# JohannesBuchner/massivedatans

Hardware: AMD Instinct MI355X
Metric: likelihood evals/sec across N datasets per constrained draw (higher is better)
Workload: dtype f64

## Files before the change

massivedatans_amd/csrc/mdns_chunk.hip:

```cpp
#include "mdns_quad.h"
#include <cstdlib>

namespace mdns {

typedef JointMailbox ChunkMailbox;

template <int NST>
__global__ __launch_bounds__(256) void k_chunk_accept(
    const double *__restrict__ Y, int ld, int nx, int nxp, const double *__restrict__ xgrid,
    const double *__restrict__ params, int B, double scale,
    const int *__restrict__ rows, int *__restrict__ rows_dev, int M, int ntiles,
    const double *__restrict__ higher, int *__restrict__ flags, int stamp, JointTrail trail, JointHeader *__restrict__ header)
{
	extern __shared__ __attribute__((aligned(16))) double lds[];
	if (blockIdx.x == 0 && threadIdx.x == 0) header->status = 0;
	double2 *tpl = reinterpret_cast<double2 *>(lds);
	double *par = lds + (size_t) nxp * 4;
	unsigned long long *votes = reinterpret_cast<unsigned long long *>(par + 12);
	const int lane = threadIdx.x & 63, wave = threadIdx.x >> 6;
	const int q = lane & 3;
	const int bt = blockIdx.x / ntiles, tile = blockIdx.x - bt * ntiles;
	double pv = 0.0;
	if (threadIdx.x < 12) {
		const int b = bt * 4 + threadIdx.x / 3;
// ... 240 lines not shown
		const int kk = live ? k : M - 1;
		const int d = thr_rows ? thr_rows[kk] : kk;
		thr[v] = live ? higher[d] : __builtin_nan("");
		yy[v] = ysq[d];
	}
	int best = 0x7fffffff;
#pragma unroll
	for (int c = 0; c < NC; c++) {
		const int cand = (ct0 + c) * 16 + i;
		const bool valid = ct0 + c < nbt && cand < B;
		const double mm = msq[valid ? cand : 0];
		bool hit = false, maybe = false;
#pragma unroll
		for (int v = 0; v < 4; v++) {
			const double S = acc[c][v];
			const double Lf = scale * ((mm - 2.0 * S) + yy[v]);
			const double E4 = 4.0 * unit * ((mm + 2.0 * fabs(S)) + yy[v]);
			const bool h = valid && Lf > thr[v] + E4;
			hit = hit || h;
			maybe = maybe || (valid && !h && Lf >= thr[v] - E4);
		}
		const unsigned long long hm = __ballot(hit), mb = __ballot(maybe);
		if (lane < 16) {
			const unsigned long long mine = 0x0001000100010001ull << lane;
			if (hm & mine) { flags[cand] = 1; best = cand < best ? cand : best; }
			else if (mb & mine) ambiguous[cand] = stamp;
		}
	}
#pragma unroll
	for (int off = 8; off > 0; off >>= 1) { const int o = __shfl_xor(best, off, 64); best = o < best ? o : best; }
	if (lane == 0 && best != 0x7fffffff) atomicMax(lowest, B - best);
}

template <int NC, bool KSPLIT>
__global__ __launch_bounds__(256) void k_gauss_gemm_filter(
    const double *__restrict__ YG, int nxg, int nx, const double *__restrict__ model_g, const double *__restrict__ msq, int B,
    double scale, const int *__restrict__ thr_rows, int M, int nbt,
    const double *__restrict__ higher, const double *__restrict__ ysq, int *__restrict__ flags, int *__restrict__ ambiguous,
    int stamp, int *__restrict__ lowest)
{
	__shared__ double red[KSPLIT ? 3 : 1][KSPLIT ? NC * 256 : 1];
	const int lane = threadIdx.x & 63, wave = __builtin_amdgcn_readfirstlane((int) (threadIdx.x >> 6));
	const int i = lane & 15, q = lane >> 4;
	const int rtile = KSPLIT ? blockIdx.x : blockIdx.x * 4 + wave;
	const int first = rtile * 16;
	if (first >= M) return;
	const int ct0 = blockIdx.y * NC;
	const int ncp = nxg >> 1, ng = nxg >> 4;
	const int g0 = KSPLIT ? (wave * ng) >> 2 : 0, g1 = KSPLIT ? ((wave + 1) * ng) >> 2 : ng;
	const double *pa = YG + (((size_t) rtile * ncp + 2 * q) << 5) + 2 * i;
	const double *pb[NC];
#pragma unroll
	for (int c = 0; c < NC; c++) pb[c] = model_g + (((size_t) (ct0 + c < nbt ? ct0 + c : nbt - 1) * ncp + 2 * q) << 5) + 2 * i;
	double4_t acc[NC];
#pragma unroll
	for (int c = 0; c < NC; c++) acc[c] = double4_t{0, 0, 0, 0};
	double4_t a[2], b[2][NC];
#define GG_LOAD4(P, G) gg_join(*reinterpret_cast<const double2_t *>((P) + ((size_t) (G) << 8)), *reinterpret_cast<const double2_t *>((P) + ((size_t) (G) << 8) + 32))
#define GG_FETCH(SET, G) { \
	const int g_ = (G) < g1 ? (G) : g1 - 1; \
	a[SET] = GG_LOAD4(pa, g_); \
	_Pragma("unroll") for (int c = 0; c < NC; c++) b[SET][c] = GG_LOAD4(pb[c], g_); }
#define GG_BODY(SET, G) { \
	__builtin_amdgcn_sched_barrier(0); \
	if ((G) < g1) { \
		_Pragma("unroll") for (int t = 0; t < 4; t++) \
			_Pragma("unroll") for (int c = 0; c < NC; c++) \
				acc[c] = __builtin_amdgcn_mfma_f64_16x16x4f64(a[SET][t], b[SET][c][t], acc[c], 0, 0, 0); \
	} \
	__builtin_amdgcn_sched_barrier(0); }
	if (g0 < g1) {
		GG_FETCH(0, g0)
// ... 24 lines not shown
				acc[c][v] = ((acc[c][v] + red[0][(c * 4 + v) * 64 + lane]) + red[1][(c * 4 + v) * 64 + lane]) + red[2][(c * 4 + v) * 64 + lane];
	}
	const double unit = fabs(scale) * (double) (nx + 8) * 0x1p-52;
	double thr[4], yy[4];
#pragma unroll
	for (int v = 0; v < 4; v++) {
		const int k = first + 4 * v + q;
		const bool live = k < M;
		const int kk = live ? k : M - 1;
		const int d = thr_rows ? thr_rows[kk] : kk;
		thr[v] = live ? higher[d] : __builtin_nan("");
		yy[v] = ysq[d];
	}
	int best = 0x7fffffff;
#pragma unroll
	for (int c = 0; c < NC; c++) {
		const int cand = (ct0 + c) * 16 + i;
		const bool valid = ct0 + c < nbt && cand < B;
		const double mm = msq[valid ? cand : 0];
		bool hit = false, maybe = false;
#pragma unroll
		for (int v = 0; v < 4; v++) {
			const double S = acc[c][v];
			const double Lf = scale * ((mm - 2.0 * S) + yy[v]);
			const double E4 = 4.0 * unit * ((mm + 2.0 * fabs(S)) + yy[v]);
			const bool h = valid && Lf > thr[v] + E4;
			hit = hit || h;
			maybe = maybe || (valid && !h && Lf >= thr[v] - E4);
		}
		const unsigned long long hm = __ballot(hit), mb = __ballot(maybe);
		if (lane < 16) {
			const unsigned long long mine = 0x0001000100010001ull << lane;
			if (hm & mine) { flags[cand] = 1; best = cand < best ? cand : best; }
			else if (mb & mine) ambiguous[cand] = stamp;
		}
	}
#pragma unroll
	for (int off = 8; off > 0; off >>= 1) { const int o = __shfl_xor(best, off, 64); best = o < best ? o : best; }
	if (lane == 0 && best != 0x7fffffff) atomicMax(lowest, B - best);
}

static constexpr int kExactMost = 64;
template <int NST>
__global__ __launch_bounds__(256) void k_exact_list(
    const double *__restrict__ Y, int ld, int nxp, const double *__restrict__ model_t, double scale,
    const int *__restrict__ rows, int M, int ntiles, const double *__restrict__ higher, int B,
    const int *__restrict__ ambiguous, int stamp, const int *__restrict__ lowest, int *__restrict__ flags, JointTrail trail,
    JointHeader *__restrict__ header)
{
	extern __shared__ __attribute__((aligned(16))) double lds[];
	double2 *tpl = reinterpret_cast<double2 *>(lds);
	unsigned long long *votes = reinterpret_cast<unsigned long long *>(lds + (size_t) nxp * 4);
	__shared__ int list[kExactMost];
	__shared__ int s_n;
	const int lane = threadIdx.x & 63, wave = threadIdx.x >> 6;
	if (wave == 0) {
		const int low = *lowest > 0 ? B - *lowest : B;
		int n = 0;
		for (int b0 = 0; b0 < B && b0 <= low; b0 += 64) {
			const int b = b0 + lane;
			const bool take = b < B && ((b < low && ambiguous[b] == stamp) || b == low);
			const unsigned long long m = __ballot(take);
			if (take) {
				const int at = n + __popcll(m & ((1ull << lane) - 1ull));
				if (at < kExactMost) list[at] = b;
			}
			n += __popcll(m);
		}
		if (lane == 0) {
			s_n = n < kExactMost ? n : kExactMost;
			if (n > kExactMost && blockIdx.x == 0) atomicOr(&header->status, 2);
		}
	}
	__syncthreads();
	const int n = s_n;
	if (n == 0) return;
	const int q = lane & 3;
	const int tile = blockIdx.x;
	const int r = wave * 16 + (lane >> 2);
	const int k = tile * 64 + r;
	const bool live = k < M;
	const int kk = live ? k : M - 1;
	const int row = rows ? rows[kk] : kk;
	double2 y[NST];
	const double thr = quad_load_row<NST>(Y, ld, row, live, q, higher, y);
	for (int g = 0; g < n; g += 4) {
		quad_templates_listed(lds, model_t, nxp, list, g, n);
		__syncthreads();
		const double L = quad_sum<NST>(tpl, nxp / kCH, q, y) * scale;
		const bool has_q = g + q < n, has_w = g + wave < n;
		quad_vote(L, thr, has_q, has_q ? list[g + q] : -1, has_w, has_w ? list[g + wave] : -1, ntiles, tile, r, votes, flags, 1, trail);
		__syncthreads();
	}
}

bool chunk_fits(const mdns_spectra *s, int M, int B)
{
	Context *c = ctx();
	const int ntiles = (M + 63) / 64;
	const long long groups = (long long) ntiles * ((B + 3) / 4);
	static const char *limit = getenv("MDNS_CHUNK_GROUPS");
	const long long most = limit && atoll(limit) > 0 ? atoll(limit) : 16LL * c->num_cus;
	if (M > 4096 && B > 8) return false;
	return groups <= most && cols_nx(s->nx) <= 8 * 32 && s->d_x != nullptr;
}

bool launch_chunk_accept(const mdns_spectra *s, const double *d_params_mapped, int B, double scale,
                         const int *d_rows_in, int *d_rows_dev, int M, const double *d_higher,
                         int *d_flags, int stamp, const JointTrail &trail, void *d_header)
{
	Context *c = ctx();
	const int ntiles = (M + 63) / 64;
	const int nbt = (B + 3) / 4;
	const int nxp = cols_nx(s->nx);
	const size_t lds = ((size_t) nxp * 4 + 12 + 4) * sizeof(double);
	const int nst = nxp / kCH;
	ProfileScope prof(0);
#define CHUNK_LAUNCH(NST) hipLaunchKernelGGL((k_chunk_accept<NST>), dim3(ntiles * nbt), dim3(256), lds, c->stream, \
	s->d_y, s->ld, s->nx, nxp, s->d_x, d_params_mapped, B, scale, d_rows_in, d_rows_dev, M, ntiles, d_higher, d_flags, stamp, trail, (JointHeader *) d_header)
	if (nst <= 8) { note_kernel(0, "k_chunk_accept<8>"); CHUNK_LAUNCH(8); }
	else if (nst <= 16) { note_kernel(0, "k_chunk_accept<16>"); CHUNK_LAUNCH(16); }
	else if (nst <= 26) { note_kernel(0, "k_chunk_accept<26>"); CHUNK_LAUNCH(26); }
	else { note_kernel(0, "k_chunk_accept<32>"); CHUNK_LAUNCH(32); }
#undef CHUNK_LAUNCH
	return launched("k_chunk_accept");
}

bool launch_chunk_commit(const int *d_thr_rows, int M, int B, const int *d_flags, int stamp, const JointTrail &trail,
                         const JointArrays &st, void *d_header, unsigned long long *d_fillbits, void *box_dev,
                         unsigned long long seq)
{
	Context *c = ctx();
	const int ntiles = (M + 63) / 64;
	hipLaunchKernelGGL(k_chunk_commit, dim3(1), dim3(1024), 0, c->stream, d_thr_rows, M, B, ntiles, d_flags, stamp, trail, st,
	                   (JointHeader *) d_header, d_fillbits, (ChunkMailbox *) box_dev, seq);
	return launched("k_chunk_commit");
}

int gauss_mfma_form()
{
	static int form = -1;
	if (form < 0) {
		const char *e = getenv("MDNS_K1_FILTER_FORM");
		form = e && e[0] == 'd' ? 1 : (e && e[0] == 'l' ? 0 : 2);
	}
	return form;
}

bool launch_gauss_mfma_filter(const mdns_spectra *s, const double *d_yT, const double *d_model_t, int B, double scale,
                              const int *d_thr_rows, int M, const double *d_higher, int *d_flags,
                              const double *d_msq, const JointTrail &trail, int *d_lowest, int *d_scratch, void *d_header,
                              const double *d_yG, const double *d_model_g)
{
	Context *c = ctx();
	const int ntiles = (M + 63) / 64, nbt = (B + 15) / 16;
	const int nxp = cols_nx(s->nx);
	int *d_amb = d_scratch;
	{
		static const char *probe = getenv("MDNS_FILTER_PROBE");
		const int pr = probe ? atoi(probe) : 0;
		if (pr == 0 && d_yG && d_model_g && gauss_mfma_form() == 2) {
			const int nxg = tiled16_nx(s->nx);
			static const char *ncf = getenv("MDNS_K1_GEMM_NC");
			int nc = nbt >= 2 ? 2 : 1;
			if (ncf && (atoi(ncf) == 1 || atoi(ncf) == 2 || atoi(ncf) == 4) && atoi(ncf) <= nbt) nc = atoi(ncf);
			ProfileScope prof(0);
			note_kernel(0, "k_gauss_gemm_filter<%d>", nc);
			static const char *ks = getenv("MDNS_K1_GEMM_KSPLIT");
			const bool ksplit = ks && ks[0] == '1';
			const int rt = (M + 15) / 16;
#define GG_LAUNCH(NC) do { if (ksplit) hipLaunchKernelGGL((k_gauss_gemm_filter<NC, true>), dim3(rt, (nbt + NC - 1) / NC), dim3(256), 0, c->stream, \
			d_yG, nxg, s->nx, d_model_g, d_msq, B, scale, d_thr_rows, M, nbt, d_higher, (const double *) s->d_ysq, d_flags, d_amb, trail.stamp, d_lowest); \
		else hipLaunchKernelGGL((k_gauss_gemm_filter<NC, false>), dim3((rt + 3) / 4, (nbt + NC - 1) / NC), dim3(256), 0, c->stream, \
			d_yG, nxg, s->nx, d_model_g, d_msq, B, scale, d_thr_rows, M, nbt, d_higher, (const double *) s->d_ysq, d_flags, d_amb, trail.stamp, d_lowest); } while (0)
			if (nc == 4) GG_LAUNCH(4); else if (nc == 2) GG_LAUNCH(2); else GG_LAUNCH(1);
#undef GG_LAUNCH
			if (!launched("k_gauss_gemm_filter")) return false;
		} else if (pr == 0 && gauss_mfma_form() == 1) {
			static double *d_zeros = nullptr;
			if (!d_zeros && (!MDNS_HIP(hipMalloc((void **) &d_zeros, 16 * sizeof(double))) ||
			                 !MDNS_HIP(hipMemsetAsync(d_zeros, 0, 16 * sizeof(double), c->stream)))) return false;
			const int nc = nbt >= 16 ? 4 : (nbt >= 8 ? 2 : 1);
			const int gy = (nbt + 4 * nc - 1) / (4 * nc);
			ProfileScope prof(0);
			note_kernel(0, "k_gauss_mfma_direct<%d>", nc);
#define GD_LAUNCH(NC) hipLaunchKernelGGL((k_gauss_mfma_direct<NC>), dim3((M + 15) / 16, gy), dim3(256), 0, c->stream, \
			d_yT, nxp, s->nx, d_model_t, d_msq, B, scale, d_thr_rows, M, nbt, d_higher, (const double *) s->d_ysq, d_flags, d_amb, trail.stamp, d_lowest, \
			(const double *) d_zeros)
			if (nc == 4) GD_LAUNCH(4); else if (nc == 2) GD_LAUNCH(2); else GD_LAUNCH(1);
#undef GD_LAUNCH
			if (!launched("k_gauss_mfma_direct")) return false;
		} else {
		const int nspec = (M + 31) / 32;
		const int ngroups = (nbt + 3) / 4;
		const int blocks = 8 * ((nspec + 7) / 8) * ngroups;
		ProfileScope prof(0);
		note_kernel(0, "k_gauss_mfma_filter");
#define MFMA_LAUNCH(D, P) hipLaunchKernelGGL((k_gauss_mfma_filter<32, 32, D, P>), dim3(blocks), dim3(256), 0, c->stream, \
		                   d_yT, nxp, s->nx, d_model_t, d_msq, B, scale, d_thr_rows, M, nspec, nbt, ngroups, d_higher, \
		                   (const double *) s->d_ysq, d_flags, d_amb, trail.stamp, d_lowest)
		const bool forty = pr == 0 && (nxp + 39) / 40 * 40 < (nxp + 31) / 32 * 32;
		if (forty) hipLaunchKernelGGL((k_gauss_mfma_filter<32, 40, 1, 0>), dim3(blocks), dim3(256), 0, c->stream,
		                              d_yT, nxp, s->nx, d_model_t, d_msq, B, scale, d_thr_rows, M, nspec, nbt, ngroups, d_higher,
		                              (const double *) s->d_ysq, d_flags, d_amb, trail.stamp, d_lowest);
		else switch (pr) {
		case 1: MFMA_LAUNCH(1, 1); break;
		case 2: MFMA_LAUNCH(1, 2); break;
		case 3: MFMA_LAUNCH(1, 3); break;
		case 4: MFMA_LAUNCH(2, 0); break;
		case 5: MFMA_LAUNCH(1, 0); break;
// ... 18 lines not shown
```

massivedatans_amd/csrc/mdns_internal.h:

```cpp
#pragma once
#include <hip/hip_runtime.h>
#include <cstddef>
#include <cstdint>
#include "mdns.h"

namespace mdns {

void set_error(const char *fmt, ...);
bool hip_ok(hipError_t e, const char *what, const char *file, int line);
#define MDNS_HIP(call) ::mdns::hip_ok((call), #call, __FILE__, __LINE__)
bool launched(const char *name);

enum class Wait { ok, timeout, failed, empty };
Wait wait_seq(const volatile unsigned long long *at, unsigned long long want, hipError_t *err = nullptr);

struct Context {
	int device = -1;
	hipStream_t own_stream = nullptr;
	hipStream_t stream = nullptr;
	int num_cus = 256;
	void *d_ws = nullptr;   size_t d_ws_bytes = 0;
	void *h_pin = nullptr;  size_t h_pin_bytes = 0;
	void *d_mask = nullptr; size_t d_mask_bytes = 0;
};
// ... 54 lines not shown
	int *stamp_of;
	unsigned long long *word;
	double *L;
	int stamp;
};
struct JointMailbox { unsigned long long seq; int accepted; int status; unsigned long long bits[1];  };
bool chunk_fits(const mdns_spectra *s, int M, int B);
bool launch_chunk_accept(const mdns_spectra *s, const double *d_params_mapped, int B, double scale,
                         const int *d_rows_in, int *d_rows_dev, int M, const double *d_higher,
                         int *d_flags, int stamp, const JointTrail &trail, void *d_header);
bool launch_chunk_commit(const int *d_thr_rows, int M, int B, const int *d_flags, int stamp, const JointTrail &trail,
                         const JointArrays &st, void *d_header, unsigned long long *d_fillbits, void *box_dev,
                         unsigned long long seq);
bool launch_gauss_cols_accept(const mdns_spectra *s, const double *d_yT, const double *d_model_t, int bt, int B,
                              double scale, const int *d_rows, const int *d_thr_rows, int M,
                              const double *d_higher, int *d_flags, const JointTrail &trail);
int gauss_filter_pays(const mdns_spectra *s, int M, int B);
int gauss_filter_tile(int M, int B);
bool launch_gauss_model_tsq(const double *d_x, int nx, const double *d_params, int B, int bt, double *d_model_t, double *d_msq,
                            int *d_zero, int nzero, double *d_model_g = nullptr);
bool launch_gauss_cols_filter(const mdns_spectra *s, const double *d_yT, const double *d_model_t, int bt, int B,
                              double scale, const int *d_rows, const int *d_thr_rows, int M,
                              const double *d_higher, int *d_flags, const double *d_msq, const JointTrail &trail, int *d_lowest);
bool launch_row_sumsq(const double *d_y, int ld, int nx, int ndata, double *d_out);
#ifdef __HIPCC__
__host__ __device__
#endif
inline size_t tiled16_at(size_t r, int c, int ncp) { return (((r >> 4) * (size_t) ncp + (size_t) (c >> 1)) << 5) + ((r & 15) << 1) + (size_t) (c & 1); }
inline int tiled16_nx(int nx) { return (nx + 15) & ~15; }
bool launch_tile_rows16(const double *d_y, int ld, int M, int nx, const int *d_rows, double *d_out);
bool launch_gauss_mfma_filter(const mdns_spectra *s, const double *d_yT, const double *d_model_t, int B, double scale,
                              const int *d_thr_rows, int M, const double *d_higher, int *d_flags,
                              const double *d_msq, const JointTrail &trail, int *d_lowest, int *d_scratch, void *d_header,
                              const double *d_yG = nullptr, const double *d_model_g = nullptr);
int gauss_mfma_form();
bool launch_joint_commit_trail(const int *d_thr_rows, int M, int B, const int *d_flags, const JointTrail &trail,
                               const JointArrays &st, void *d_header, unsigned long long *d_fillbits, int flag_value = 1,
                               void *box_dev = nullptr, unsigned long long seq = 0, int *d_ticket = nullptr);
bool launch_gauss_cols_commit(const mdns_spectra *s, const double *d_yT, const double *d_model_t, int mstride, int B,
                              double scale, const int *d_rows, const int *d_thr_rows, int M, const int *d_flags,
                              const JointArrays &st, void *d_header, unsigned long long *d_fillbits, double *d_Lrow);
bool launch_gauss_cols(const mdns_spectra *s, const double *d_yT, const double *d_model_t, int bt, int B,
                       double scale, const int *d_rows, int M, double *d_out);
bool launch_muse3_model(const double *d_x, int nx, const double *d_params, int B,
                        double *d_model, int ldm);
bool launch_gauss_rows(const mdns_spectra *s, const double *d_model, int ldm, int B,
                       double scale, const int *d_rows, int M, double *d_out);
struct MuseBandFused;
bool launch_muse_rows(const mdns_spectra *s, const double *d_model, int ldm, int B,
                      const int *d_rows, int M, double *d_out, int B_shape = 0, const MuseBandFused *band = nullptr);
int muse_rows_variant(int B, int M);
struct MuseBandOut { int *counter, *clear, *maybe, *pair_b, *pair_k; double *pair_L, *pair_thr; int cap; int *zero_at; };
bool muse_filter_applies(const mdns_spectra *s, int B, int M);
int muse_filter_ld(int nx);
bool launch_muse_filter(mdns_spectra *s, const double *d_model, int ldm, int B, const int *d_rows, int M,
                        const double *d_higher, const double *d_bound, const MuseBandOut &out);
void muse_filter_note(int which);
bool launch_transpose(const double *d_src, int nx, int ndata, double *d_dst, int ld,
                      bool invert, int lds);
bool launch_tile_columns(const double *d_y, int ld, int ndata, int nx, const int *d_rows, double *d_yt);
bool launch_copy_rows(const double *d_src, int nx, int ndata, double *d_dst, int ld,
                      bool invert);
bool launch_pad_model(const double *d_src, int nx, int B, double *d_dst, int ldm);

struct RegionResult {
	double radius;
	double thresh;
	unsigned long long seq;
	unsigned long long pad;
};
struct BootstrapFinish {
	unsigned *counter;
	RegionResult *d_res;
	RegionResult *h_res;
// ... 179 lines not shown
```

massivedatans_amd/csrc/mdns_joint.hip:

```cpp
#include "mdns_internal.h"

#include <cmath>
#include <cstring>
#include <vector>

namespace mdns {

static constexpr int kBlock = 256;
static constexpr int kFlagInts = MDNS_JOINT_MAX_BATCH;
static constexpr int kZeroInts = kFlagInts + (int) (sizeof(JointHeader) / sizeof(int));

static constexpr int kSlices = 16, kHeld = 8;

template <typename T, typename F> __device__ __forceinline__ T over_slices(T v, F f)
{
	v = f(v, __shfl_xor(v, 4));
	v = f(v, __shfl_xor(v, 8));
	v = f(v, __shfl_xor(v, 16));
	v = f(v, __shfl_xor(v, 32));
	return v;
}

__global__ __launch_bounds__(kBlock) void k_joint_prepare(JointArrays st, const int *__restrict__ running, int nrun,
                                                          double *__restrict__ Lmin, int *__restrict__ argmin_run,
// ... 258 lines not shown
__global__ void k_joint_fill(double *__restrict__ p, size_t n, double value)
{
	for (size_t e = (size_t) blockIdx.x * blockDim.x + threadIdx.x; e < n; e += (size_t) gridDim.x * blockDim.x) p[e] = value;
}

}

using namespace mdns;

struct ChunkScore { int path, B, flag; };

struct mdns_joint {
	mdns_spectra *s = nullptr;
	int nlive = 0, cap = 0, ndata = 0;
	JointArrays st = {};
	int *d_running = nullptr;  int nrun = 0;
	double *d_Lmin = nullptr;
	int *d_argmin_run = nullptr;
	int *d_argmin = nullptr;
	unsigned long long *d_keep = nullptr;  size_t keep_cap = 0;
	int *d_status = nullptr;
	int *d_flags = nullptr;
	char *d_result = nullptr;
	JointMailbox *h_box = nullptr, *h_box_dev = nullptr;
	unsigned long long box_seq = 0;
	bool box_pending = false;
	int *d_trail_stamp = nullptr;  unsigned long long *d_trail_word = nullptr;  double *d_trail_L = nullptr;
	size_t trail_cap = 0;
	int trail_stamp = 0;
	bool trail_valid = false;
	double *d_params = nullptr;
	int *d_rows = nullptr;
	char *h_pin = nullptr;  size_t pin_bytes = 0;
	const double *last_yT = nullptr;
	const int *last_gather = nullptr;
	int last_bt = 0, last_B = 0;
	double last_scale = 0;
	bool prepared = false;
	bool staged_rows = false;
	bool staged_valid = false;
	int scored_M = -1;
	int staged_M = 0;
	size_t staged_in_bytes = 0;
	double noise_level = 0;
	int kind = 0;
	int nparams = 3;
	double *d_msq = nullptr;
	int *d_filter_scratch = nullptr;
	double *d_dense = nullptr;  size_t dense_cap = 0;
	double *d_jitter = nullptr;  size_t jitter_cap = 0;
	int *d_sel_rows = nullptr;  size_t sel_rows_cap = 0;
	bool sel_rows = false;
	int sel_M = 0;
	bool sel_open = false;
	bool sel_on_device = false;
	int chunk_seq = 1;
	char *h_in = nullptr, *h_in_dev = nullptr;
	int shelf_bound = 0;
	ChainBox *h_chain = nullptr, *h_chain_dev = nullptr;
	double *d_chain_props = nullptr;
	int *d_chain_counts = nullptr, *d_chain_ticket = nullptr;
	int *d_commit_ticket = nullptr;
	BandBox *h_band = nullptr, *h_band_dev = nullptr;
	BandScratch *d_band = nullptr;
	double *d_bound = nullptr;
	unsigned long long band_seq = 0;
	int band_B = 0;
	bool band_pending = false;
// ... 370 lines not shown
		if (filter == 2 && gauss_mfma_form() == 2 && (d_row_ids || s->d_yG)) {
			const size_t need = (size_t) ((B + 15) / 16) * 16 * tiled16_nx(s->nx);
			if (need > s->model_g_cap) {
				if (s->d_model_g) { if (!joint_sync(c)) return 1; (void) hipFree(s->d_model_g); s->d_model_g = nullptr; s->model_g_cap = 0; }
				if (!MDNS_HIP(hipMalloc((void **) &s->d_model_g, (need + need / 2) * sizeof(double)))) return 1;
				s->model_g_cap = need + need / 2;
			}
			model_g = s->d_model_g;
		}
		if (!launch_gauss_model_tsq(s->d_x, s->nx, d_params, B, bt, s->d_model, j->d_msq, j->d_flags, kZeroInts, model_g)) return 1;
		gemm_form = model_g != nullptr;
	} else if (!launch_gauss_model_t(s->d_x, s->nx, d_params, B, bt, s->d_model, j->d_flags, kZeroInts)) return 1;
	const double *yT = s->d_yT;
	const int *gather = d_row_ids;
	const bool sparse = (size_t) M * 8 < (size_t) s->ndata;
	const double *yG = s->d_yG;
	if (d_row_ids && gemm_form) {
		const size_t need = (size_t) ((M + 15) / 16) * 16 * tiled16_nx(s->nx);
		if (need > s->selG_cap) {
			if (s->d_selG) { if (!joint_sync(c)) return 1; (void) hipFree(s->d_selG); s->d_selG = nullptr; s->selG_cap = 0; }
			if (!MDNS_HIP(hipMalloc((void **) &s->d_selG, (need + need / 2) * sizeof(double)))) return 1;
			s->selG_cap = need + need / 2;
		}
		if (!launch_tile_rows16(s->d_y, s->ld, M, s->nx, d_row_ids, s->d_selG)) return 1;
		yG = s->d_selG;
	} else if (d_row_ids && (B >= 128 || sparse || filter == 2)) {
		if (!ensure_selection(s, (size_t) ((M + 63) / 64) * 64 * cols_nx(s->nx))) return 1;
		if (!launch_tile_columns(s->d_y, s->ld, M, s->nx, d_row_ids, s->d_sel)) return 1;
		yT = s->d_sel;
		gather = nullptr;
	}
	JointTrail trail;
	if (!joint_trail(j, B, M, &trail)) return 1;
	if (filter == 2) {
		int *lowest = (int *) &((JointHeader *) j->d_result)->pad;
		if (!launch_gauss_mfma_filter(s, yT, s->d_model, B, scale, d_row_ids, M, j->st.higher, j->d_flags, j->d_msq, trail, lowest,
		                              j->d_filter_scratch, j->d_result, gemm_form ? yG : nullptr, gemm_form ? s->d_model_g : nullptr)) return 1;
	} else if (filter) {
		int *lowest = (int *) &((JointHeader *) j->d_result)->pad;
		if (!launch_gauss_cols_filter(s, yT, s->d_model, bt, B, scale, gather, d_row_ids, M, j->st.higher, j->d_flags, j->d_msq, trail, lowest)) return 1;
	} else if (!launch_gauss_cols_accept(s, yT, s->d_model, bt, B, scale, gather, d_row_ids, M, j->st.higher, j->d_flags, trail)) return 1;
	j->trail_valid = true;
	j->last_yT = yT; j->last_gather = gather; j->last_bt = bt; j->last_B = B; j->last_scale = scale;
	j->scored_M = M;
	return 0;
}

extern "C" int *mdns_joint_flags_dev(mdns_joint *j) { return j ? j->d_flags : nullptr; }
extern "C" const void *mdns_joint_result_dev(mdns_joint *j) { return j ? j->d_result : nullptr; }

static bool commit_ticket(mdns_joint *j)
{
	if (j->d_commit_ticket) return true;
	Context *c = ctx();
	return MDNS_HIP(hipMalloc((void **) &j->d_commit_ticket, sizeof(int))) && MDNS_HIP(hipMemsetAsync(j->d_commit_ticket, 0, sizeof(int), c->stream));
}

static unsigned long long *result_bits(const mdns_joint *j) { return (unsigned long long *) (j->d_result + sizeof(JointHeader)); }

static void launch_publish(mdns_joint *j, Context *c, int M)
{
	hipLaunchKernelGGL(k_joint_publish, dim3(1), dim3(kBlock), 0, c->stream, (const JointHeader *) j->d_result, result_bits(j), (M + 63) / 64,
	                   j->h_box_dev, ++j->box_seq);
}

static bool commit_from_trail(mdns_joint *j, const int *thr_rows, int M, int B, const int *decides, int value, bool one_group)
{
	const JointTrail trail = {j->d_trail_stamp, j->d_trail_word, j->d_trail_L, j->trail_stamp};
	if (one_group && M <= 128) {
		return launch_chunk_commit(thr_rows, M, B, decides, value, trail, j->st, j->d_result, result_bits(j), j->h_box_dev, ++j->box_seq);
	}
	return commit_ticket(j) && launch_joint_commit_trail(thr_rows, M, B, decides, trail, j->st, j->d_result, result_bits(j), value, j->h_box_dev,
	                                                     ++j->box_seq, j->d_commit_ticket);
}

static int joint_commit_dev(mdns_joint *j, const int *d_row_ids, int M, bool want_row, const char *who)
{
	Context *c = ctx();
	if (!c || !check_draw(j, 0, M, who)) return 1;
	if (j->scored_M != M) {
		set_error("%s: M=%d, but the score that precedes had M=%d (-1: none, or already committed)", who, M, j->scored_M);
		return 1;
	}
	j->scored_M = -1;
	if (j->last_B == 0 || M == 0) {
		static const JointHeader none = {-1, 0, 0};
		if (!MDNS_HIP(hipMemcpyAsync(j->d_result, &none, sizeof none, hipMemcpyHostToDevice, c->stream)) || !joint_sync(c)) return 1;
		j->h_box->accepted = -1; j->h_box->status = 0;
		j->h_box->seq = ++j->box_seq;
		j->box_pending = true;
		return 0;
	}
	if (!want_row && j->trail_valid) {
		if (!commit_from_trail(j, d_row_ids, M, j->last_B, j->d_flags, 1, false)) return 1;
	} else {
		double *Lrow = (double *) (j->d_result + sizeof(JointHeader) + (size_t) ((M + 63) / 64) * 8);
		if (!launch_gauss_cols_commit(j->s, j->last_yT, j->s->d_model, j->last_bt, j->last_B, j->last_scale, j->last_gather,
		                              d_row_ids, M, j->d_flags, j->st, j->d_result, result_bits(j), Lrow)) return 1;
		launch_publish(j, c, M);
	}
	j->trail_valid = false;
	j->box_pending = true;
	return MDNS_HIP(hipGetLastError()) ? 0 : 1;
}

extern "C" int mdns_joint_commit_dev(mdns_joint *j, const int *d_row_ids, int M)
{
	return joint_commit_dev(j, d_row_ids, M, true, "mdns_joint_commit_dev");
}

extern "C" int mdns_joint_commit_bits_dev(mdns_joint *j, const int *d_row_ids, int M)
{
	return joint_commit_dev(j, d_row_ids, M, false, "mdns_joint_commit_bits_dev");
}

static bool joint_wait_box(mdns_joint *j, const char *who)
{
	if (!j->box_pending) { set_error("%s: no commit to wait for", who); return false; }
	hipError_t e = hipSuccess;
	switch (wait_seq(&j->h_box->seq, j->box_seq, &e)) {
	case Wait::ok: break;
	case Wait::timeout: set_error("%s: no outcome within MDNS_POLL_TIMEOUT_S", who); return false;
	case Wait::failed: set_error("%s: the commit failed: %s", who, hipGetErrorString(e)); return false;
	case Wait::empty: set_error("%s: the commit finished without an outcome", who); return false;
	}
	j->box_pending = false;
	return true;
}

static int joint_read_box(mdns_joint *j, int M, int *accepted, unsigned long long *fillbits, const char *who)
{
	if (!joint_wait_box(j, who)) return 1;
// ... 616 lines not shown
```

massivedatans_amd/csrc/mdns_like.hip:

```cpp
#include "mdns_internal.h"
#include <climits>
#include <cstdlib>

namespace mdns {

static constexpr int kBlock = 256;

template <int CTRL, int ROW_MASK>
__device__ __forceinline__ double dpp_move(double v)
{
	const int lo = __builtin_amdgcn_update_dpp(0, __double2loint(v), CTRL, ROW_MASK, 0xf, true);
	const int hi = __builtin_amdgcn_update_dpp(0, __double2hiint(v), CTRL, ROW_MASK, 0xf, true);
	return __hiloint2double(hi, lo);
}

__device__ __forceinline__ double wave_sum(double v)
{
	v += dpp_move<0xb1, 0xf>(v);
	v += dpp_move<0x4e, 0xf>(v);
	v += dpp_move<0x114, 0xf>(v);
	v += dpp_move<0x118, 0xf>(v);
	v += dpp_move<0x142, 0xa>(v);
	v += dpp_move<0x143, 0xc>(v);
	const int lo = __builtin_amdgcn_readlane(__double2loint(v), 63);
// ... 550 lines not shown
	__shared__ int s_first;
	__shared__ int s_last;
	const int bstar = first_flagged<kBlock>(&s_first, flags, B, [=](int f) { return f == flag_value; });
	if (blockIdx.x == 0 && threadIdx.x == 0) header->accepted = bstar < B ? bstar : -1;
	const int lane = threadIdx.x & 63;
	const int tile = blockIdx.x * (kBlock / 64) + (threadIdx.x >> 6);
	const bool mine = bstar < B && tile < ntiles;
	if (!mine && !box) return;
	const size_t at = mine ? (size_t) bstar * ntiles + tile : 0;
	const unsigned long long word = mine && trail.stamp_of[at] == trail.stamp ? trail.word[at] : 0ull;
	const int k = tile * 64 + lane;
	if (mine && k < M && (word >> lane & 1ull)) {
		const int d = thr_rows ? thr_rows[k] : k;
		if (!shelf_append<25>(st, d, trail.L[at * 64 + lane], st.higher[d])) atomicOr(&header->status, 1);
	}
	if (!box) { if (lane == 0) fillbits[tile] = word; return; }
	if (mine && lane == 0) __hip_atomic_store(&fillbits[tile], word, __ATOMIC_RELAXED, __HIP_MEMORY_SCOPE_AGENT);
	handover_release();
	__syncthreads();
	if (threadIdx.x == 0) s_last = atomicAdd(ticket, 1) == (int) gridDim.x - 1 ? 1 : 0;
	__syncthreads();
	if (!s_last) return;
	handover_acquire();
	if (bstar < B)
		for (int w = threadIdx.x; w < ntiles; w += kBlock)
			mail_store(&box->bits[w], __hip_atomic_load(&fillbits[w], __ATOMIC_RELAXED, __HIP_MEMORY_SCOPE_AGENT));
	handover_release();
	__syncthreads();
	if (threadIdx.x != 0) return;
	*ticket = 0;
	mail_store(&box->accepted, bstar < B ? bstar : -1);
	mail_store(&box->status, __hip_atomic_load(&header->status, __ATOMIC_RELAXED, __HIP_MEMORY_SCOPE_AGENT));
	mail_raise(&box->seq, seq);
}

__global__ __launch_bounds__(kBlock) void k_gauss_cols_commit(
    const double *__restrict__ YT, int nxp, const double *__restrict__ model_t, int mstride, int B,
    double scale, const int *__restrict__ rows, const int *__restrict__ thr_rows, int M,
    int ntiles, int nq_xcd, int cu_slots, const int *__restrict__ flags, JointArrays st,
    JointHeader *__restrict__ header, unsigned long long *__restrict__ fillbits, double *__restrict__ Lrow)
{
	extern __shared__ __attribute__((aligned(16))) double tpl[];
	const int bstar = first_flagged<kBlock>(reinterpret_cast<int *>(tpl + nxp), flags, B, [](int f) { return f != 0; });
	if (blockIdx.x == 0 && threadIdx.x == 0) header->accepted = bstar < B ? bstar : -1;
	if (bstar >= B) return;
	const int lane = threadIdx.x & 63;
	int tile, bt_unused;
	if (!cols_item(ntiles, INT_MAX, nq_xcd, 1, cu_slots, tile, bt_unused)) return;
	stage_templates(tpl, model_t + (size_t) (bstar / mstride) * nxp * mstride + bstar % mstride, nxp, mstride);
	if (tile >= ntiles) return;
	int k[1];
	double acc[1][1];
	cols_accumulate_deep<1, 4>(YT, nxp, tpl, rows, M, tile, lane, k[0], acc[0]);
	const bool live = k[0] < M;
	const double L = acc[0][0] * scale;
	bool beats = false;
	if (live) {
		const int d = thr_rows ? thr_rows[k[0]] : k[0];
		Lrow[k[0]] = L;
		const double thr = st.higher[d];
		beats = L > thr;
		if (beats && !shelf_append<8>(st, d, L, thr)) atomicOr(&header->status, 1);
	}
	const unsigned long long word = __ballot(beats);
	if (lane == 0) fillbits[tile] = word;
}

template <int BT>
__global__ __launch_bounds__(kBlock) void k_gauss_rows_generic(
    const double *__restrict__ Y, int ld, int nx, const double *__restrict__ model, int ldm, int B,
    double scale, const int *__restrict__ rows, int M, double *__restrict__ out)
{
	const int lane = threadIdx.x & 63;
	const int wave = (blockIdx.x * kBlock + threadIdx.x) >> 6;
	const int nwaves = (gridDim.x * kBlock) >> 6;
	const int ch = 2 * lane;
	for (int k = wave; k < M; k += nwaves) {
		const int row = rows ? rows[k] : k;
		const double *yr = Y + (size_t) row * ld;
		for (int b0 = 0; b0 < B; b0 += BT) {
			double acc[BT];
#pragma unroll
			for (int b = 0; b < BT; b++) acc[b] = 0.0;
			for (int c0 = 0; c0 < nx; c0 += 128) {
				const bool ok = c0 + ch < nx;
				const double2 yv = ok ? *reinterpret_cast<const double2 *>(yr + c0 + ch) : make_double2(0.0, 0.0);
#pragma unroll
				for (int b = 0; b < BT; b++) {
					const int bb = (b0 + b < B) ? b0 + b : B - 1;
					const double2 mv = *reinterpret_cast<const double2 *>(model + (size_t) bb * ldm + c0 + ch);
					const double d0 = mv.x - yv.x, d1 = mv.y - yv.y;
					acc[b] = fma(d0, d0, acc[b]);
					acc[b] = fma(d1, d1, acc[b]);
				}
			}
#pragma unroll
			for (int b = 0; b < BT; b++) {
				const double s = wave_sum(acc[b]);
// ... 348 lines not shown
		    !MDNS_HIP(hipMemsetAsync(d_tickets, 0, (size_t) cap * sizeof(int), c->stream))) return false;
		cap_tiles = cap;
	}
	hipLaunchKernelGGL(k_gauss_model_tsq, dim3(ntile, ny), dim3(256), 0, c->stream, d_x, nx, cols_nx(nx), d_params, B, bt, d_model_t, d_msq,
	                   d_zero, d_zero ? nzero : 0, d_model_g, tiled16_nx(nx), d_part, d_tickets);
	return launched("k_gauss_model_tsq");
}

bool launch_tile_rows16(const double *d_y, int ld, int M, int nx, const int *d_rows, double *d_out)
{
	Context *c = ctx();
	if (M <= 0 || nx <= 0) return true;
	hipLaunchKernelGGL(k_tile_rows16, dim3((M + 15) / 16), dim3(256), 0, c->stream, d_y, ld, M, nx, tiled16_nx(nx), d_rows, d_out);
	return launched("k_tile_rows16");
}

bool launch_gauss_cols_filter(const mdns_spectra *s, const double *d_yT, const double *d_model_t, int bt, int B,
                              double scale, const int *d_rows, const int *d_thr_rows, int M,
                              const double *d_higher, int *d_flags, const double *d_msq, const JointTrail &trail, int *d_lowest)
{
	Context *c = ctx();
	const int ntiles = (M + 63) / 64;
	const int nbt = (B + bt - 1) / bt;
	const int nxp = cols_nx(s->nx);
	int nq_xcd, cu_slots;
	const int blocks = cols_grid(c, ntiles, nbt, nq_xcd, cu_slots, 4);
	ProfileScope prof(0);
	note_kernel(0, "k_gauss_cols_filter<%d>", bt);
#define FILTER_LAUNCH(BT) hipLaunchKernelGGL((k_gauss_cols_filter<BT>), dim3(blocks), dim3(256), 0, c->stream, \
	d_yT, nxp, s->nx, d_model_t, d_msq, B, scale, d_rows, d_thr_rows, M, ntiles, nq_xcd, nbt, cu_slots, d_higher, (const double *) s->d_ysq, d_flags, trail, d_lowest)
	if (bt == 16) FILTER_LAUNCH(16); else FILTER_LAUNCH(8);
#undef FILTER_LAUNCH
	return launched("k_gauss_cols_filter");
}

bool launch_gauss_cols_commit(const mdns_spectra *s, const double *d_yT, const double *d_model_t, int mstride, int B,
                              double scale, const int *d_rows, const int *d_thr_rows, int M, const int *d_flags,
                              const JointArrays &st, void *d_header, unsigned long long *d_fillbits, double *d_Lrow)
{
	Context *c = ctx();
	const int ntiles = (M + 63) / 64;
	int nq_xcd, cu_slots;
	const int blocks = cols_grid(c, ntiles, 1, nq_xcd, cu_slots);
	hipLaunchKernelGGL(k_gauss_cols_commit, dim3(blocks), dim3(kBlock), (size_t) (cols_nx(s->nx) + 2) * sizeof(double), c->stream,
	                   d_yT, cols_nx(s->nx), d_model_t, mstride, B, scale, d_rows, d_thr_rows, M, ntiles, nq_xcd, cu_slots,
	                   d_flags, st, (JointHeader *) d_header, d_fillbits, d_Lrow);
	return launched("k_gauss_cols_commit");
}

bool launch_joint_commit_trail(const int *d_thr_rows, int M, int B, const int *d_flags, const JointTrail &trail,
                               const JointArrays &st, void *d_header, unsigned long long *d_fillbits, int flag_value,
                               void *box_dev, unsigned long long seq, int *d_ticket)
{
	Context *c = ctx();
	const int ntiles = (M + 63) / 64;
	hipLaunchKernelGGL(k_joint_commit_trail, dim3((ntiles + kBlock / 64 - 1) / (kBlock / 64)), dim3(kBlock), 0, c->stream,
	                   d_thr_rows, M, B, ntiles, d_flags, flag_value, trail, st, (JointHeader *) d_header, d_fillbits,
	                   (JointMailbox *) box_dev, seq, d_ticket);
	return launched("k_joint_commit_trail");
}

bool launch_muse3_model(const double *d_x, int nx, const double *d_params, int B, double *d_model, int ldm)
{
	Context *c = ctx();
	dim3 grid((ldm + kBlock * kMuseModelPer - 1) / (kBlock * kMuseModelPer), B);
	hipLaunchKernelGGL(k_muse3_model, grid, dim3(kBlock), 0, c->stream, d_x, nx, d_params, d_model, ldm);
	return launched("k_muse3_model");
}

bool launch_pad_model(const double *d_src, int nx, int B, double *d_dst, int ldm)
{
	Context *c = ctx();
	dim3 grid((ldm + kBlock - 1) / kBlock, B);
	hipLaunchKernelGGL(k_pad_model, grid, dim3(kBlock), 0, c->stream, d_src, nx, d_dst, ldm);
	return launched("k_pad_model");
}

bool launch_transpose(const double *d_src, int nx, int ndata, double *d_dst, int ld, bool invert, int lds)
{
	Context *c = ctx();
// ... 115 lines not shown
```

massivedatans_amd/csrc/mdns_quad.h:

```cpp
#pragma once
#include "mdns_internal.h"

#ifdef __HIPCC__
namespace mdns {

static constexpr int kCH = 8;

template <int Q>
__device__ __forceinline__ double quad_bcast(double v)
{
	constexpr int ctrl = Q | (Q << 2) | (Q << 4) | (Q << 6);
	const int lo = __builtin_amdgcn_update_dpp(0, __double2loint(v), ctrl, 0xf, 0xf, true);
	const int hi = __builtin_amdgcn_update_dpp(0, __double2hiint(v), ctrl, 0xf, 0xf, true);
	return __hiloint2double(hi, lo);
}

template <int NST>
__device__ __forceinline__ double quad_load_row(const double *__restrict__ Y, int ld, int row, bool live, int q,
                                                const double *__restrict__ higher, double2 (&y)[NST])
{
	const double *yr = Y + (size_t) row * ld;
#pragma unroll
	for (int s = 0; s < NST; s++) {
		const int j = s * kCH + 2 * q;
		const double2 v = *reinterpret_cast<const double2 *>(yr + (j < ld ? j : 0));
		y[s].x = j < ld ? v.x : 0.0;
		y[s].y = j < ld ? v.y : 0.0;
	}
	return live ? higher[row] : __builtin_nan("");
}

__device__ __forceinline__ void quad_templates(double *__restrict__ tpl, const double *__restrict__ par,
                                               const double *__restrict__ xgrid, int nx, int nxp, int first, int B)
{
	for (int e = threadIdx.x; e < nxp * 4; e += 256) {
		const int j = e >> 2, bb = e & 3;
		double m = 0.0;
		if (j < nx && first + bb < B) {
			const double A = par[bb * 3], mu = par[bb * 3 + 1], sig = par[bb * 3 + 2];
			const double t = (mu - xgrid[j]) / sig;
			m = A * exp(-0.5 * (t * t));
		}
		tpl[((size_t) (j >> 1) * 4 + bb) * 2 + (j & 1)] = m;
	}
}

__device__ __forceinline__ void quad_templates_listed(double *__restrict__ tpl, const double *__restrict__ model_t, int nxp,
                                                      const int *__restrict__ list, int g, int n)
{
	for (int e = threadIdx.x; e < nxp * 4; e += 256) {
		const int j = e >> 2, bb = e & 3;
		const int c = g + bb < n ? list[g + bb] : -1;
		const double m = c >= 0 ? model_t[((size_t) (c >> 4) * nxp + j) * 16 + (c & 15)] : 0.0;
		tpl[((size_t) (j >> 1) * 4 + bb) * 2 + (j & 1)] = m;
	}
}

template <int NST>
__device__ __forceinline__ double quad_sum(const double2 *__restrict__ tpl, int nst, int q, const double2 (&y)[NST])
{
	double acc = 0.0;
#pragma unroll
	for (int s = 0; s < NST; s++) {
		if (s < nst) {
			const double2 *m = tpl + (size_t) s * 16 + q;
			double d;
#define QUARTER(QQ) { const double2 mv = m[QQ * 4]; \
			d = mv.x - quad_bcast<QQ>(y[s].x); acc = fma(d, d, acc); \
			d = mv.y - quad_bcast<QQ>(y[s].y); acc = fma(d, d, acc); }
			QUARTER(0) QUARTER(1) QUARTER(2) QUARTER(3)
#undef QUARTER
		}
	}
	return acc;
}

__device__ __forceinline__ void quad_vote(double L, double thr, bool has_q, int cand_q, bool has_w, int cand_w, int ntiles, int tile,
                                          int r, unsigned long long *votes, int *__restrict__ flags, int flag, const JointTrail &trail)
{
	const int lane = threadIdx.x & 63, wave = threadIdx.x >> 6;
	const bool beat = L > thr && has_q;
	const unsigned long long vote = __ballot(beat);
	if (lane == 0) votes[wave] = vote;
	if (beat) trail.L[((size_t) cand_q * ntiles + tile) * 64 + r] = L;
	__syncthreads();
	const unsigned long long word = __ballot((votes[lane >> 4] >> (4 * (lane & 15) + wave)) & 1ull);
	if (has_w && word != 0ull && lane == 0) {
		const size_t at = (size_t) cand_w * ntiles + tile;
		flags[cand_w] = flag;
		trail.word[at] = word;
		trail.stamp_of[at] = trail.stamp;
	}
}

}
#endif
```

Measured before the change: 29.01 billion.

## Resolve ambiguous GEMM-filter candidates inline and add fused commit-score kernel with mailbox

The GEMM filter now recomputes the exact likelihood for ambiguous candidates inside the filter kernel, instead of marking them for a separate exact-list pass. When the GEMM path is taken it reports that no trail was left, so the commit recomputes scores for the accepted draw. That commit goes through a new quad-layout kernel that also does the mailbox handoff via a last-block ticket, replacing the cols commit kernel plus a separate publish launch. The goal is fewer kernel launches and passes. The cost is a serial, uncoalesced per-candidate exact loop inside the filter and a recompute at commit time.

```diff
diff --git a/massivedatans_amd/csrc/mdns_chunk.hip b/massivedatans_amd/csrc/mdns_chunk.hip
--- a/massivedatans_amd/csrc/mdns_chunk.hip
+++ b/massivedatans_amd/csrc/mdns_chunk.hip
@@ -296,12 +296,37 @@
 	if (lane == 0 && best != 0x7fffffff) atomicMax(lowest, B - best);
 }
 
+struct GemmExact {
+	const double *Y; int ld;
+	const double *model_t; int nxp;
+};
+__device__ __forceinline__ void gemm_resolve(GemmExact ex, int nx, double scale, const int *__restrict__ thr_rows, int M,
+                                                       const double *__restrict__ higher, int first, int cand, int B,
+                                                       int *__restrict__ flags, int *__restrict__ lowest)
+{
+	const int lane = threadIdx.x & 63;
+	const int k = first + (lane & 15);
+	const bool live = k < M;
+	const int kk = live ? k : M - 1;
+	const int row = thr_rows ? thr_rows[kk] : kk;
+	const double *yr = ex.Y + (size_t) row * ex.ld;
+	const double *mp = ex.model_t + (size_t) (cand >> 4) * ex.nxp * 16 + (cand & 15);
+	double acc = 0.0;
+#pragma unroll 8
+	for (int j = 0; j < nx; j++) {
+		const double d = mp[(size_t) j * 16] - yr[j];
+		acc = fma(d, d, acc);
+	}
+	const double L = acc * scale;
+	if (__ballot(live && L > higher[row]) != 0ull && lane == 0) { flags[cand] = 1; atomicMax(lowest, B - cand); }
+}
+
 template <int NC, bool KSPLIT>
 __global__ __launch_bounds__(256) void k_gauss_gemm_filter(
     const double *__restrict__ YG, int nxg, int nx, const double *__restrict__ model_g, const double *__restrict__ msq, int B,
     double scale, const int *__restrict__ thr_rows, int M, int nbt,
-    const double *__restrict__ higher, const double *__restrict__ ysq, int *__restrict__ flags, int *__restrict__ ambiguous,
-    int stamp, int *__restrict__ lowest)
+    const double *__restrict__ higher, const double *__restrict__ ysq, int *__restrict__ flags, GemmExact exact,
+    int *__restrict__ lowest)
 {
 	__shared__ double red[KSPLIT ? 3 : 1][KSPLIT ? NC * 256 : 1];
 	const int lane = threadIdx.x & 63, wave = __builtin_amdgcn_readfirstlane((int) (threadIdx.x >> 6));
@@ -392,7 +417,13 @@
 		if (lane < 16) {
 			const unsigned long long mine = 0x0001000100010001ull << lane;
 			if (hm & mine) { flags[cand] = 1; best = cand < best ? cand : best; }
-			else if (mb & mine) ambiguous[cand] = stamp;
+		}
+		unsigned todo = (unsigned) ((mb | mb >> 16 | mb >> 32 | mb >> 48) & ~(hm | hm >> 16 | hm >> 32 | hm >> 48) & 0xffffull);
+#pragma unroll 1
+		while (todo) {
+			const int t = __builtin_ctz(todo);
+			todo &= todo - 1;
+			gemm_resolve(exact, nx, scale, thr_rows, M, higher, first, (ct0 + c) * 16 + t, B, flags, lowest);
 		}
 	}
 #pragma unroll
@@ -454,6 +485,70 @@
 	}
 }
 
+template <int NST>
+__global__ __launch_bounds__(256) void k_joint_commit_score(
+    const double *__restrict__ Y, int ld, int nxp, const double *__restrict__ model_t, int mstride, double scale,
+    const int *__restrict__ rows, int M, int ntiles, int B, const int *__restrict__ flags, JointArrays st,
+    JointHeader *__restrict__ header, unsigned long long *__restrict__ fillbits, double *__restrict__ Lrow,
+    JointMailbox *__restrict__ box, unsigned long long seq, int *__restrict__ ticket)
+{
+	extern __shared__ __attribute__((aligned(16))) double lds[];
+	double *tpl = lds;
+	unsigned long long *votes = reinterpret_cast<unsigned long long *>(lds + nxp);
+	__shared__ int s_first, s_last;
+	const int bstar = first_flagged<256>(&s_first, flags, B, [](int f) { return f != 0; });
+	if (blockIdx.x == 0 && threadIdx.x == 0) header->accepted = bstar < B ? bstar : -1;
+	const int lane = threadIdx.x & 63, wave = threadIdx.x >> 6;
+	const int tile = blockIdx.x;
+	if (bstar < B) {
+		const int q = lane & 3;
+		const int r = wave * 16 + (lane >> 2);
+		const int k = tile * 64 + r;
+		const bool live = k < M;
+		const int kk = live ? k : M - 1;
+		const int row = rows ? rows[kk] : kk;
+		const int nst = nxp / kCH;
+		double2 y[NST];
+		const double thr = quad_load_row<NST>(Y, ld, row, live, q, st.higher, y);
+		const double *mp = model_t + (size_t) (bstar / mstride) * nxp * mstride + bstar % mstride;
+		for (int e = threadIdx.x; e < nxp; e += 256) tpl[e] = mp[(size_t) e * mstride];
+		__syncthreads();
+		double acc = quad_sum_one<NST>(tpl, nst, y, 0.0);
+		for (int s0 = NST; s0 < nst; s0 += NST) {
+			quad_load_row<NST>(Y, ld, row, live, q, st.higher, y, s0);
+			acc = quad_sum_one<NST>(tpl + (size_t) s0 * kCH, nst - s0, y, acc);
+		}
+		const double L = acc * scale;
+		const bool mine = live && q == 0;
+		if (mine && Lrow) Lrow[k] = L;
+		const bool beats = mine && L > thr;
+		if (beats && !shelf_append<25>(st, row, L, thr)) atomicOr(&header->status, 1);
+		const unsigned long long vote = __ballot(beats);
+		if (lane == 0) votes[wave] = vote;
+		__syncthreads();
+		if (wave == 0) {
+			const unsigned long long word = __ballot((votes[lane >> 4] >> (4 * (lane & 15))) & 1ull);
+			if (lane == 0) __hip_atomic_store(&fillbits[tile], word, __ATOMIC_RELAXED, __HIP_MEMORY_SCOPE_AGENT);
+		}
+	}
+	handover_release();
+	__syncthreads();
+	if (threadIdx.x == 0) s_last = atomicAdd(ticket, 1) == (int) gridDim.x - 1 ? 1 : 0;
+	__syncthreads();
+	if (!s_last) return;
+	handover_acquire();
+	if (bstar < B)
+		for (int w = threadIdx.x; w < ntiles; w += 256)
+			mail_store(&box->bits[w], __hip_atomic_load(&fillbits[w], __ATOMIC_RELAXED, __HIP_MEMORY_SCOPE_AGENT));
+	handover_release();
+	__syncthreads();
+	if (threadIdx.x != 0) return;
+	*ticket = 0;
+	mail_store(&box->accepted, bstar < B ? bstar : -1);
+	mail_store(&box->status, __hip_atomic_load(&header->status, __ATOMIC_RELAXED, __HIP_MEMORY_SCOPE_AGENT));
+	mail_raise(&box->seq, seq);
+}
+
 bool chunk_fits(const mdns_spectra *s, int M, int B)
 {
 	Context *c = ctx();
@@ -497,6 +592,24 @@
 	return launched("k_chunk_commit");
 }
 
+bool launch_joint_commit_score(const mdns_spectra *s, const double *d_model_t, int mstride, int B, double scale,
+                               const int *d_rows, int M, const int *d_flags, const JointArrays &st, void *d_header,
+                               unsigned long long *d_fillbits, double *d_Lrow, void *box_dev, unsigned long long seq, int *d_ticket)
+{
+	Context *c = ctx();
+	const int ntiles = (M + 63) / 64;
+	const int nxp = cols_nx(s->nx);
+	const size_t lds = ((size_t) nxp + 4) * sizeof(double);
+	if (lds > 64 * 1024) { set_error("launch_joint_commit_score: %d channels do not fit the commit's LDS", s->nx); return false; }
+	const int nst = nxp / kCH;
+#define COMMIT_LAUNCH(NST) hipLaunchKernelGGL((k_joint_commit_score<NST>), dim3(ntiles), dim3(256), lds, c->stream, \
+	s->d_y, s->ld, nxp, d_model_t, mstride, scale, d_rows, M, ntiles, B, d_flags, st, (JointHeader *) d_header, d_fillbits, d_Lrow, \
+	(JointMailbox *) box_dev, seq, d_ticket)
+	if (nst <= 8) COMMIT_LAUNCH(8); else if (nst <= 16) COMMIT_LAUNCH(16); else if (nst <= 26) COMMIT_LAUNCH(26); else COMMIT_LAUNCH(32);
+#undef COMMIT_LAUNCH
+	return launched("k_joint_commit_score");
+}
+
 int gauss_mfma_form()
 {
 	static int form = -1;
@@ -510,9 +623,10 @@
 bool launch_gauss_mfma_filter(const mdns_spectra *s, const double *d_yT, const double *d_model_t, int B, double scale,
                               const int *d_thr_rows, int M, const double *d_higher, int *d_flags,
                               const double *d_msq, const JointTrail &trail, int *d_lowest, int *d_scratch, void *d_header,
-                              const double *d_yG, const double *d_model_g)
+                              bool *left_trail, const double *d_yG, const double *d_model_g)
 {
 	Context *c = ctx();
+	*left_trail = true;
 	const int ntiles = (M + 63) / 64, nbt = (B + 15) / 16;
 	const int nxp = cols_nx(s->nx);
 	int *d_amb = d_scratch;
@@ -529,13 +643,15 @@
 			static const char *ks = getenv("MDNS_K1_GEMM_KSPLIT");
 			const bool ksplit = ks && ks[0] == '1';
 			const int rt = (M + 15) / 16;
+			const GemmExact exact = {s->d_y, s->ld, d_model_t, nxp};
 #define GG_LAUNCH(NC) do { if (ksplit) hipLaunchKernelGGL((k_gauss_gemm_filter<NC, true>), dim3(rt, (nbt + NC - 1) / NC), dim3(256), 0, c->stream, \
-			d_yG, nxg, s->nx, d_model_g, d_msq, B, scale, d_thr_rows, M, nbt, d_higher, (const double *) s->d_ysq, d_flags, d_amb, trail.stamp, d_lowest); \
+			d_yG, nxg, s->nx, d_model_g, d_msq, B, scale, d_thr_rows, M, nbt, d_higher, (const double *) s->d_ysq, d_flags, exact, d_lowest); \
 		else hipLaunchKernelGGL((k_gauss_gemm_filter<NC, false>), dim3((rt + 3) / 4, (nbt + NC - 1) / NC), dim3(256), 0, c->stream, \
-			d_yG, nxg, s->nx, d_model_g, d_msq, B, scale, d_thr_rows, M, nbt, d_higher, (const double *) s->d_ysq, d_flags, d_amb, trail.stamp, d_lowest); } while (0)
+			d_yG, nxg, s->nx, d_model_g, d_msq, B, scale, d_thr_rows, M, nbt, d_higher, (const double *) s->d_ysq, d_flags, exact, d_lowest); } while (0)
 			if (nc == 4) GG_LAUNCH(4); else if (nc == 2) GG_LAUNCH(2); else GG_LAUNCH(1);
 #undef GG_LAUNCH
-			if (!launched("k_gauss_gemm_filter")) return false;
+			*left_trail = false;
+			return launched("k_gauss_gemm_filter");
 		} else if (pr == 0 && gauss_mfma_form() == 1) {
 			static double *d_zeros = nullptr;
 			if (!d_zeros && (!MDNS_HIP(hipMalloc((void **) &d_zeros, 16 * sizeof(double))) ||
diff --git a/massivedatans_amd/csrc/mdns_internal.h b/massivedatans_amd/csrc/mdns_internal.h
--- a/massivedatans_amd/csrc/mdns_internal.h
+++ b/massivedatans_amd/csrc/mdns_internal.h
@@ -110,14 +110,14 @@
 bool launch_gauss_mfma_filter(const mdns_spectra *s, const double *d_yT, const double *d_model_t, int B, double scale,
                               const int *d_thr_rows, int M, const double *d_higher, int *d_flags,
                               const double *d_msq, const JointTrail &trail, int *d_lowest, int *d_scratch, void *d_header,
-                              const double *d_yG = nullptr, const double *d_model_g = nullptr);
+                              bool *left_trail, const double *d_yG = nullptr, const double *d_model_g = nullptr);
 int gauss_mfma_form();
 bool launch_joint_commit_trail(const int *d_thr_rows, int M, int B, const int *d_flags, const JointTrail &trail,
                                const JointArrays &st, void *d_header, unsigned long long *d_fillbits, int flag_value = 1,
                                void *box_dev = nullptr, unsigned long long seq = 0, int *d_ticket = nullptr);
-bool launch_gauss_cols_commit(const mdns_spectra *s, const double *d_yT, const double *d_model_t, int mstride, int B,
-                              double scale, const int *d_rows, const int *d_thr_rows, int M, const int *d_flags,
-                              const JointArrays &st, void *d_header, unsigned long long *d_fillbits, double *d_Lrow);
+bool launch_joint_commit_score(const mdns_spectra *s, const double *d_model_t, int mstride, int B, double scale,
+                               const int *d_rows, int M, const int *d_flags, const JointArrays &st, void *d_header,
+                               unsigned long long *d_fillbits, double *d_Lrow, void *box_dev, unsigned long long seq, int *d_ticket);
 bool launch_gauss_cols(const mdns_spectra *s, const double *d_yT, const double *d_model_t, int bt, int B,
                        double scale, const int *d_rows, int M, double *d_out);
 bool launch_muse3_model(const double *d_x, int nx, const double *d_params, int B,
diff --git a/massivedatans_amd/csrc/mdns_joint.hip b/massivedatans_amd/csrc/mdns_joint.hip
--- a/massivedatans_amd/csrc/mdns_joint.hip
+++ b/massivedatans_amd/csrc/mdns_joint.hip
@@ -314,8 +314,6 @@
 	double *d_params = nullptr;
 	int *d_rows = nullptr;
 	char *h_pin = nullptr;  size_t pin_bytes = 0;
-	const double *last_yT = nullptr;
-	const int *last_gather = nullptr;
 	int last_bt = 0, last_B = 0;
 	double last_scale = 0;
 	bool prepared = false;
@@ -752,16 +750,17 @@
 	}
 	JointTrail trail;
 	if (!joint_trail(j, B, M, &trail)) return 1;
+	bool left_trail = true;
 	if (filter == 2) {
 		int *lowest = (int *) &((JointHeader *) j->d_result)->pad;
 		if (!launch_gauss_mfma_filter(s, yT, s->d_model, B, scale, d_row_ids, M, j->st.higher, j->d_flags, j->d_msq, trail, lowest,
-		                              j->d_filter_scratch, j->d_result, gemm_form ? yG : nullptr, gemm_form ? s->d_model_g : nullptr)) return 1;
+		                              j->d_filter_scratch, j->d_result, &left_trail, gemm_form ? yG : nullptr, gemm_form ? s->d_model_g : nullptr)) return 1;
 	} else if (filter) {
 		int *lowest = (int *) &((JointHeader *) j->d_result)->pad;
 		if (!launch_gauss_cols_filter(s, yT, s->d_model, bt, B, scale, gather, d_row_ids, M, j->st.higher, j->d_flags, j->d_msq, trail, lowest)) return 1;
 	} else if (!launch_gauss_cols_accept(s, yT, s->d_model, bt, B, scale, gather, d_row_ids, M, j->st.higher, j->d_flags, trail)) return 1;
-	j->trail_valid = true;
-	j->last_yT = yT; j->last_gather = gather; j->last_bt = bt; j->last_B = B; j->last_scale = scale;
+	j->trail_valid = left_trail;
+	j->last_bt = bt; j->last_B = B; j->last_scale = scale;
 	j->scored_M = M;
 	return 0;
 }
@@ -814,10 +813,10 @@
 	if (!want_row && j->trail_valid) {
 		if (!commit_from_trail(j, d_row_ids, M, j->last_B, j->d_flags, 1, false)) return 1;
 	} else {
-		double *Lrow = (double *) (j->d_result + sizeof(JointHeader) + (size_t) ((M + 63) / 64) * 8);
-		if (!launch_gauss_cols_commit(j->s, j->last_yT, j->s->d_model, j->last_bt, j->last_B, j->last_scale, j->last_gather,
-		                              d_row_ids, M, j->d_flags, j->st, j->d_result, result_bits(j), Lrow)) return 1;
-		launch_publish(j, c, M);
+		double *Lrow = want_row ? (double *) (j->d_result + sizeof(JointHeader) + (size_t) ((M + 63) / 64) * 8) : nullptr;
+		if (!commit_ticket(j) ||
+		    !launch_joint_commit_score(j->s, j->s->d_model, j->last_bt, j->last_B, j->last_scale, d_row_ids, M, j->d_flags, j->st,
+		                               j->d_result, result_bits(j), Lrow, j->h_box_dev, ++j->box_seq, j->d_commit_ticket)) return 1;
 	}
 	j->trail_valid = false;
 	j->box_pending = true;
diff --git a/massivedatans_amd/csrc/mdns_like.hip b/massivedatans_amd/csrc/mdns_like.hip
--- a/massivedatans_amd/csrc/mdns_like.hip
+++ b/massivedatans_amd/csrc/mdns_like.hip
@@ -606,38 +606,6 @@
 	mail_store(&box->accepted, bstar < B ? bstar : -1);
 	mail_store(&box->status, __hip_atomic_load(&header->status, __ATOMIC_RELAXED, __HIP_MEMORY_SCOPE_AGENT));
 	mail_raise(&box->seq, seq);
-}
-
-__global__ __launch_bounds__(kBlock) void k_gauss_cols_commit(
-    const double *__restrict__ YT, int nxp, const double *__restrict__ model_t, int mstride, int B,
-    double scale, const int *__restrict__ rows, const int *__restrict__ thr_rows, int M,
-    int ntiles, int nq_xcd, int cu_slots, const int *__restrict__ flags, JointArrays st,
-    JointHeader *__restrict__ header, unsigned long long *__restrict__ fillbits, double *__restrict__ Lrow)
-{
-	extern __shared__ __attribute__((aligned(16))) double tpl[];
-	const int bstar = first_flagged<kBlock>(reinterpret_cast<int *>(tpl + nxp), flags, B, [](int f) { return f != 0; });
-	if (blockIdx.x == 0 && threadIdx.x == 0) header->accepted = bstar < B ? bstar : -1;
-	if (bstar >= B) return;
-	const int lane = threadIdx.x & 63;
-	int tile, bt_unused;
-	if (!cols_item(ntiles, INT_MAX, nq_xcd, 1, cu_slots, tile, bt_unused)) return;
-	stage_templates(tpl, model_t + (size_t) (bstar / mstride) * nxp * mstride + bstar % mstride, nxp, mstride);
-	if (tile >= ntiles) return;
-	int k[1];
-	double acc[1][1];
-	cols_accumulate_deep<1, 4>(YT, nxp, tpl, rows, M, tile, lane, k[0], acc[0]);
-	const bool live = k[0] < M;
-	const double L = acc[0][0] * scale;
-	bool beats = false;
-	if (live) {
-		const int d = thr_rows ? thr_rows[k[0]] : k[0];
-		Lrow[k[0]] = L;
-		const double thr = st.higher[d];
-		beats = L > thr;
-		if (beats && !shelf_append<8>(st, d, L, thr)) atomicOr(&header->status, 1);
-	}
-	const unsigned long long word = __ballot(beats);
-	if (lane == 0) fillbits[tile] = word;
 }
 
 template <int BT>
@@ -1052,20 +1020,6 @@
 	if (bt == 16) FILTER_LAUNCH(16); else FILTER_LAUNCH(8);
 #undef FILTER_LAUNCH
 	return launched("k_gauss_cols_filter");
-}
-
-bool launch_gauss_cols_commit(const mdns_spectra *s, const double *d_yT, const double *d_model_t, int mstride, int B,
-                              double scale, const int *d_rows, const int *d_thr_rows, int M, const int *d_flags,
-                              const JointArrays &st, void *d_header, unsigned long long *d_fillbits, double *d_Lrow)
-{
-	Context *c = ctx();
-	const int ntiles = (M + 63) / 64;
-	int nq_xcd, cu_slots;
-	const int blocks = cols_grid(c, ntiles, 1, nq_xcd, cu_slots);
-	hipLaunchKernelGGL(k_gauss_cols_commit, dim3(blocks), dim3(kBlock), (size_t) (cols_nx(s->nx) + 2) * sizeof(double), c->stream,
-	                   d_yT, cols_nx(s->nx), d_model_t, mstride, B, scale, d_rows, d_thr_rows, M, ntiles, nq_xcd, cu_slots,
-	                   d_flags, st, (JointHeader *) d_header, d_fillbits, d_Lrow);
-	return launched("k_gauss_cols_commit");
 }
 
 bool launch_joint_commit_trail(const int *d_thr_rows, int M, int B, const int *d_flags, const JointTrail &trail,
diff --git a/massivedatans_amd/csrc/mdns_quad.h b/massivedatans_amd/csrc/mdns_quad.h
--- a/massivedatans_amd/csrc/mdns_quad.h
+++ b/massivedatans_amd/csrc/mdns_quad.h
@@ -17,12 +17,12 @@
 
 template <int NST>
 __device__ __forceinline__ double quad_load_row(const double *__restrict__ Y, int ld, int row, bool live, int q,
-                                                const double *__restrict__ higher, double2 (&y)[NST])
+                                                const double *__restrict__ higher, double2 (&y)[NST], int s0 = 0)
 {
 	const double *yr = Y + (size_t) row * ld;
 #pragma unroll
 	for (int s = 0; s < NST; s++) {
-		const int j = s * kCH + 2 * q;
+		const int j = (s0 + s) * kCH + 2 * q;
 		const double2 v = *reinterpret_cast<const double2 *>(yr + (j < ld ? j : 0));
 		y[s].x = j < ld ? v.x : 0.0;
 		y[s].y = j < ld ? v.y : 0.0;
@@ -75,6 +75,24 @@
 	return acc;
 }
 
+template <int NST>
+__device__ __forceinline__ double quad_sum_one(const double *__restrict__ tpl, int nst, const double2 (&y)[NST], double acc)
+{
+#pragma unroll
+	for (int s = 0; s < NST; s++) {
+		if (s < nst) {
+			const double2 *m = reinterpret_cast<const double2 *>(tpl) + (size_t) s * 4;
+			double d;
+#define QUARTER(QQ) { const double2 mv = m[QQ]; \
+			d = mv.x - quad_bcast<QQ>(y[s].x); acc = fma(d, d, acc); \
+			d = mv.y - quad_bcast<QQ>(y[s].y); acc = fma(d, d, acc); }
+			QUARTER(0) QUARTER(1) QUARTER(2) QUARTER(3)
+#undef QUARTER
+		}
+	}
+	return acc;
+}
+
 __device__ __forceinline__ void quad_vote(double L, double thr, bool has_q, int cand_q, bool has_w, int cand_w, int ntiles, int tile,
                                           int r, unsigned long long *votes, int *__restrict__ flags, int flag, const JointTrail &trail)
 {
```

Result: no change. 28.81 billion (-0.7%).
